# tuffy/libdvd-audio

Measured on AMD Instinct MI355X. Metric: decoded PCM Msamples/s (bit-exact) on 6ch/96k/24b MLP, higher is better.
Workload: dtype int32 (int64 accumulate)

## Files before the change

libdvd-audio_amd/csrc/mlp_hip.hip:

```cpp
#include <hip/hip_runtime.h>
#include <stdint.h>
#include <stdio.h>
#include <stdlib.h>
#include <string.h>
#include <new>
#include <vector>

#include "../../include/dvda_mlp_hip.h"
#include "mlp_step.h"
#include "mlp_decode.h"
#include "mlp_chain.h"
#include "mlp_chain_small.h"
#include "mlp_check.h"
#include "mlp_coop.h"
#include "mlp_index.h"
#include "pcm_unswizzle.h"
#include "wav_pack.h"

using namespace mlp;

#define HIP_TRY(x)                                                                         \
    do {                                                                                   \
        hipError_t e_ = (x);                                                               \
        if (e_ != hipSuccess) {                                                            \
            fprintf(stderr, "dvda_mlp_hip: %s failed: %s (%s:%d)\n", #x, hipGetErrorString(e_), \
                    __FILE__, __LINE__);                                                   \
            return DVDA_HIP_ENODEV;                                                        \
        }                                                                                  \
    } while (0)

constexpr uint32_t EV_RING = 256;
constexpr uint32_t SEQ_ROUND = 1024;

static hipError_t ws_malloc(void **p, size_t bytes)
{
    static const int poison = getenv("DVDA_POISON") ? (int)strtol(getenv("DVDA_POISON"), nullptr, 0) : -1;
    hipError_t e = hipMalloc(p, bytes);
    if (e == hipSuccess && poison >= 0)
        e = hipMemset(*p, poison & 0xFF, bytes);
    return e;
}

struct dvda_mlp_hip_ctx {
    int device;
    uint32_t coop_min_seg;
    uint32_t max_streams, max_segments;
    uint8_t *d_masks;
    uint16_t *d_parts;
    uint64_t masks_cap;
    uint32_t *d_tile_count;
    uint32_t *d_tile_base;
    uint64_t tiles_cap;
    uint64_t *d_cand_off;
    SegRec *d_seg;
    uint32_t *d_seg_frames;
    uint32_t *d_seg_fbase;
    uint32_t *d_seg_status;
    uint32_t *d_seg_rows;
    StreamRec *d_streams;
    uint32_t *d_n_cand;
    uint32_t *d_scan_tmp;
    uint64_t scan_tmp_cap;
    int32_t *d_iir;
    uint32_t *d_mat;
    unsigned long long *d_dbg;
    int32_t *d_fir;
    uint32_t *d_seg_meta;
    uint32_t *d_yield;
    uint32_t *d_seg_check;
    uint32_t *d_cls;
    uint32_t *d_shape_key;
    uint64_t *d_soff, *d_slen;
    uint32_t *d_rank;
    uint32_t *d_sorted_cnt;
    uint32_t *d_sorted_base;
    uint32_t *d_lane_seg;
    DecodeSummary *d_summary;
    DecodeSummary *h_summary;
    hipStream_t st_aux;
    hipEvent_t ev_fork, ev_join;
    uint32_t *d_seq_list;
    uint4 *d_plan;
    uint4 *d_scan4_tmp;
    uint32_t *d_def_list;
    uint32_t *d_head_list;
    uint32_t *d_chain_order;
    uint32_t *d_chain_hist;
    int32_t *d_fb;
    uint32_t fb_slots;
    uint32_t rsv_segs;
    int32_t *d_res;
    uint64_t res_cap;
    uint32_t *d_brec;
    uint64_t brec_cap;
    uint32_t *d_frec;
    uint64_t frec_cap;
    const int32_t *d_init_fir;
    uint32_t iir_lanes;
    const uint8_t *d_bytes;
    uint64_t total_bytes;
    const uint64_t *d_stream_off;
    const uint64_t *d_stream_len;
    uint32_t n_streams;
    uint64_t tiles;
    bool indexed;
    bool small_input;
    bool decoded;
    uint32_t lanes_per_seg;
    uint32_t pcm_layout;
    uint32_t chain_form;
    hipGraphExec_t idx_graph;
    const void *idx_key[4];
    uint64_t idx_key_bytes;
    uint32_t idx_key_streams;
    int idx_graph_state;
    hipEvent_t ev[2 * EV_RING];
    hipEvent_t ev_end[EV_RING];
    uint32_t ev_end_made;
    uint32_t ev_made;
    uint64_t ev_count;
};

static WsCaps ws_caps(const dvda_mlp_hip_ctx *c)
{
    WsCaps w;
    w.res = c->res_cap;
    w.brec = c->brec_cap;
    w.frec = c->frec_cap;
    w.fb = (uint64_t)c->fb_slots * FB_WORDS;
    w.max_seg = c->max_segments;
    w.max_streams = c->max_streams;
    w.lanes = c->iir_lanes;
    w.pad = 0;
    return w;
}

extern "C" int dvda_mlp_hip_bounds_violations(unsigned long long *out4)
{
    if (!out4)
        return DVDA_HIP_EINVAL;
    out4[0] = out4[1] = out4[2] = out4[3] = 0;
#if defined(DVDA_BOUNDS)
    HIP_TRY(hipDeviceSynchronize());
    HIP_TRY(hipMemcpyFromSymbol(out4, HIP_SYMBOL(mlp::g_bounds), 4 * sizeof(unsigned long long)));
    return 1;
#else
    return DVDA_HIP_OK;
#endif
}

static void free_ws(dvda_mlp_hip_ctx *c)
{
    (void)hipFree(c->d_masks);
    (void)hipFree(c->d_parts);
    (void)hipFree(c->d_tile_count);
    (void)hipFree(c->d_tile_base);
    (void)hipFree(c->d_cand_off);
    (void)hipFree(c->d_seg);
    (void)hipFree(c->d_seg_frames);
    (void)hipFree(c->d_seg_fbase);
    (void)hipFree(c->d_seg_status);
    (void)hipFree(c->d_seg_rows);
    (void)hipFree(c->d_streams);
    (void)hipFree(c->d_scan_tmp);
    (void)hipFree(c->d_iir);
    (void)hipFree(c->d_mat);
    (void)hipFree(c->d_dbg);
    (void)hipFree(c->d_fir);
    (void)hipFree(c->d_seg_meta);
    (void)hipFree(c->d_yield);
    (void)hipFree(c->d_seg_check);
    (void)hipFree(c->d_cls);
    (void)hipFree(c->d_shape_key);
    (void)hipFree(c->d_soff);
    (void)hipFree(c->d_slen);
    (void)hipFree(c->d_rank);
    (void)hipFree(c->d_sorted_cnt);
    (void)hipFree(c->d_sorted_base);
    (void)hipFree(c->d_lane_seg);
    (void)hipFree(c->d_summary);
    if (c->h_summary)
        (void)hipHostFree(c->h_summary);
    if (c->st_aux)
        (void)hipStreamDestroy(c->st_aux);
    if (c->ev_fork)
        (void)hipEventDestroy(c->ev_fork);
    if (c->ev_join)
        (void)hipEventDestroy(c->ev_join);
    (void)hipFree(c->d_seq_list);
    (void)hipFree(c->d_plan);
    (void)hipFree(c->d_scan4_tmp);
    (void)hipFree(c->d_def_list);
    (void)hipFree(c->d_head_list);
    (void)hipFree(c->d_chain_order);
    (void)hipFree(c->d_chain_hist);
    (void)hipFree(c->d_fb);
    (void)hipFree(c->d_res);
    (void)hipFree(c->d_brec);
    (void)hipFree(c->d_frec);
    for (uint32_t i = 0; i < c->ev_made; i++)
        (void)hipEventDestroy(c->ev[i]);
    for (uint32_t i = 0; i < c->ev_end_made; i++)
        (void)hipEventDestroy(c->ev_end[i]);
    if (c->idx_graph)
        (void)hipGraphExecDestroy(c->idx_graph);
}

extern "C" const char *dvda_mlp_hip_version(void) { return "dvda-mlp-hip 0.1 (gfx950)"; }

extern "C" int dvda_mlp_hip_create(dvda_mlp_hip_ctx **out, int device, uint32_t max_streams,
                                   uint32_t max_segments)
{
    if (!out || max_streams == 0 || max_segments == 0)
        return DVDA_HIP_EINVAL;
    int ndev = 0;
    if (hipGetDeviceCount(&ndev) != hipSuccess || ndev <= 0 || device < 0 || device >= ndev) {
        fprintf(stderr, "dvda_mlp_hip: no usable HIP device (count=%d, requested=%d)\n", ndev, device);
        return DVDA_HIP_ENODEV;
    }
    HIP_TRY(hipSetDevice(device));
    dvda_mlp_hip_ctx *c = new (std::nothrow) dvda_mlp_hip_ctx();
    if (!c)
        return DVDA_HIP_ENOMEM;
    c->device = device;
    {
        int cus = 0;
        if (hipDeviceGetAttribute(&cus, hipDeviceAttributeMultiprocessorCount, device) != hipSuccess || cus <= 0)
            cus = 256;
        c->coop_min_seg = (uint32_t)cus * 4u * 64u * 7u / 4u;
        if (const char *e = getenv("DVDA_COOP_MIN_SEG"))
            c->coop_min_seg = (uint32_t)strtoul(e, nullptr, 10);
    }
    c->max_streams = max_streams;
    c->max_segments = max_segments;
    c->masks_cap = 0;
    c->tiles_cap = 0;
    c->scan_tmp_cap = 0;
    c->indexed = false;
// ... 20 lines not shown
    alloc((void **)&c->d_seg_status, (ns + 4) * sizeof(uint32_t));
    alloc((void **)&c->d_seg_rows, ns * sizeof(uint32_t));
    alloc((void **)&c->d_streams, (size_t)max_streams * sizeof(StreamRec));
    c->iir_lanes = (uint32_t)(((2 * ns + DEC_THREADS - 1) / DEC_THREADS) * DEC_THREADS);
    alloc((void **)&c->d_iir, (size_t)c->iir_lanes * MAXCH * 16 * sizeof(int32_t));
    alloc((void **)&c->d_mat, (size_t)c->iir_lanes * MAXMAT * 5 * sizeof(uint32_t));
    alloc((void **)&c->d_dbg, 32 * sizeof(unsigned long long));
    alloc((void **)&c->d_fir, (size_t)c->iir_lanes * 6 * 8 * sizeof(int32_t));
    alloc((void **)&c->d_seg_meta, ((size_t)c->iir_lanes + 4) * sizeof(uint32_t));
    alloc((void **)&c->d_yield, ns * sizeof(uint32_t));
    alloc((void **)&c->d_seg_check, 2 * ns * sizeof(uint32_t));
    alloc((void **)&c->d_cls, 4 * sizeof(uint32_t));
    alloc((void **)&c->d_shape_key, (size_t)max_streams * sizeof(uint32_t));
    alloc((void **)&c->d_soff, (size_t)max_streams * sizeof(uint64_t));
    alloc((void **)&c->d_slen, (size_t)max_streams * sizeof(uint64_t));
    alloc((void **)&c->d_rank, (size_t)max_streams * sizeof(uint32_t));
    alloc((void **)&c->d_sorted_cnt, ((size_t)max_streams + 1) * sizeof(uint32_t));
    alloc((void **)&c->d_sorted_base, ((size_t)max_streams + 1) * sizeof(uint32_t));
    alloc((void **)&c->d_lane_seg, ns * sizeof(uint32_t));
    alloc((void **)&c->d_summary, (1 + SUMMARY_PARTS) * sizeof(DecodeSummary));
    alloc((void **)&c->d_seq_list, (size_t)max_streams * sizeof(uint32_t));
    alloc((void **)&c->d_plan, (ns + 5) * sizeof(uint4));
    alloc((void **)&c->d_scan4_tmp, (ns / 1024 + 4) * sizeof(uint4));
    alloc((void **)&c->d_def_list, ns * sizeof(uint32_t));
    alloc((void **)&c->d_head_list, ns * sizeof(uint32_t));
    alloc((void **)&c->d_chain_order, ns * sizeof(uint32_t));
    alloc((void **)&c->d_chain_hist, 2 * CHAIN_BUCKETS * sizeof(uint32_t));
    if (e == hipSuccess)
        e = hipHostMalloc((void **)&c->h_summary, sizeof(DecodeSummary), hipHostMallocDefault);
    if (e == hipSuccess)
        e = hipStreamCreateWithFlags(&c->st_aux, hipStreamNonBlocking);
    if (e == hipSuccess)
        e = hipEventCreateWithFlags(&c->ev_fork, hipEventDisableTiming);
    if (e == hipSuccess)
        e = hipEventCreateWithFlags(&c->ev_join, hipEventDisableTiming);
    if (e == hipSuccess)
        e = hipMemset(c->d_dbg, 0, 32 * sizeof(unsigned long long));
    if (e == hipSuccess)
        e = hipMemset(c->d_seg_meta, 0, (size_t)c->iir_lanes * sizeof(uint32_t));
    for (uint32_t i = 0; e == hipSuccess && i < 2 * EV_RING; i++) {
        e = hipEventCreate(&c->ev[i]);
        if (e == hipSuccess)
            c->ev_made = i + 1;
    }
    for (uint32_t i = 0; e == hipSuccess && i < EV_RING; i++) {
        e = hipEventCreate(&c->ev_end[i]);
        if (e == hipSuccess)
            c->ev_end_made = i + 1;
    }
    if (e != hipSuccess) {
        fprintf(stderr, "dvda_mlp_hip: workspace allocation failed: %s\n", hipGetErrorString(e));
        free_ws(c);
        delete c;
        return DVDA_HIP_ENOMEM;
    }
    *out = c;
    return DVDA_HIP_OK;
}

extern "C" void dvda_mlp_hip_destroy(dvda_mlp_hip_ctx *c)
{
    if (!c)
        return;
    (void)hipSetDevice(c->device);
#if defined(DVDA_BOUNDS)
    if (getenv("DVDA_BOUNDS_REPORT")) {
        unsigned long long v[4] = {0, 0, 0, 0};
        (void)dvda_mlp_hip_bounds_violations(v);
        fprintf(stderr, "dvda_mlp_hip: bounds violations: %llu", v[0]);
        if (v[0])
            fprintf(stderr, " (first: tag %llu index %llu capacity %llu)", v[1], v[2], v[3]);
        fprintf(stderr, "\n");
    }
#endif
    free_ws(c);
    delete c;
}

static int ensure_byte_ws(dvda_mlp_hip_ctx *c, uint64_t total_bytes)
{
    const uint64_t chunks = (total_bytes + 15) / 16 + 4;
    const uint64_t tiles = (chunks + IDX_TILE_CHUNKS - 1) / IDX_TILE_CHUNKS;
    if (chunks > c->masks_cap) {
        (void)hipFree(c->d_masks);
        (void)hipFree(c->d_parts);
        c->d_masks = nullptr;
        c->d_parts = nullptr;
        c->masks_cap = 0;
        if (ws_malloc((void **)&c->d_masks, chunks) != hipSuccess ||
            ws_malloc((void **)&c->d_parts, (chunks + 72) * sizeof(uint16_t)) != hipSuccess)
            return DVDA_HIP_ENOMEM;
        c->masks_cap = chunks;
    }
    {
        uint64_t most = tiles > c->max_segments ? tiles : c->max_segments;
        if (c->max_streams > most)
            most = c->max_streams;
        const uint64_t need = (most + 1023) / 1024 + 2;
        if (need > c->scan_tmp_cap) {
            (void)hipFree(c->d_scan_tmp);
            c->d_scan_tmp = nullptr;
            c->scan_tmp_cap = 0;
            if (ws_malloc((void **)&c->d_scan_tmp, need * sizeof(uint32_t)) != hipSuccess)
                return DVDA_HIP_ENOMEM;
            c->scan_tmp_cap = need;
        }
    }
    if (tiles > c->tiles_cap) {
        (void)hipFree(c->d_tile_count);
        (void)hipFree(c->d_tile_base);
        c->d_tile_count = c->d_tile_base = nullptr;
        c->tiles_cap = 0;
        if (ws_malloc((void **)&c->d_tile_count, (tiles + 1) * sizeof(uint32_t)) != hipSuccess ||
            ws_malloc((void **)&c->d_tile_base, (tiles + 1) * sizeof(uint32_t)) != hipSuccess)
            return DVDA_HIP_ENOMEM;
        c->tiles_cap = tiles;
    }
    return DVDA_HIP_OK;
}

static void exscan(dvda_mlp_hip_ctx *c, hipStream_t st, const uint32_t *in, uint32_t *out, uint32_t n_host,
                   const uint32_t *n_ptr, uint32_t n_cap)
{
    const uint32_t n_max = n_ptr ? n_cap : n_host;
    if (n_max <= 4096) {
        hipLaunchKernelGGL(k_exscan_u32, dim3(1), dim3(1024), 0, st, in, out, n_host, n_ptr, n_cap);
        return;
    }
    const uint32_t blocks = (n_max + 1023) / 1024;
    hipLaunchKernelGGL(k_scan_blocks, dim3(blocks), dim3(1024), 0, st, in, out, c->d_scan_tmp, n_host, n_ptr,
                       n_cap);
    hipLaunchKernelGGL(k_exscan_u32, dim3(1), dim3(1024), 0, st, c->d_scan_tmp, c->d_scan_tmp, blocks,
                       (const uint32_t *)nullptr, blocks);
    hipLaunchKernelGGL(k_scan_add, dim3(blocks), dim3(1024), 0, st, out, c->d_scan_tmp, blocks, n_host, n_ptr,
                       n_cap);
}

__global__ void k_init_streams(StreamRec *s, uint32_t n, uint32_t *seg_status, uint32_t *seg_rows, uint32_t *yield_req,
                               uint32_t *seg_meta, uint32_t n_seg, uint32_t *cls, uint32_t *summary_words)
{
    const uint32_t i = blockIdx.x * blockDim.x + threadIdx.x;
    if (i < 4)
        cls[i] = 0;
    if (i < (1 + SUMMARY_PARTS) * sizeof(DecodeSummary) / sizeof(uint32_t))
        summary_words[i] = 0;
    if (i < n_seg) {
        seg_status[i] = 0;
        seg_rows[i] = 0;
        yield_req[i] = 0;
        seg_meta[2 * (size_t)i] = seg_meta[2 * (size_t)i + 1] = 0;
    }
    if (i < n) {
        StreamRec r;
        r.first_seg = 0xFFFFFFFFu;
        r.n_seg = 0;
        r.sync = 0;
        r.status = 0;
        r.frames = 0;
        r.consumed = 0;
        r.rows = 0;
        s[i] = r;
    }
}

__global__ void k_reset_segments(uint32_t *seg_status, uint32_t *seg_rows, uint32_t *yield_req, uint32_t *seg_meta,
                                 uint32_t n_seg)
{
    const uint32_t i = blockIdx.x * blockDim.x + threadIdx.x;
    if (i < n_seg) {
        seg_status[i] = 0;
        seg_rows[i] = 0;
        yield_req[i] = 0;
        seg_meta[2 * (size_t)i] = seg_meta[2 * (size_t)i + 1] = 0;
    }
}

__device__ __forceinline__ void check_ranges_block(const uint64_t *__restrict__ off, const uint64_t *__restrict__ len,
                                                   uint32_t n, uint64_t total_bytes, uint64_t *__restrict__ soff,
                                                   uint64_t *__restrict__ slen, StreamRec *__restrict__ streams,
                                                   unsigned long long *s_max)
{
    const uint32_t per = (n + 1023u) / 1024u;
    const uint32_t lo = threadIdx.x * per, hi = lo + per < n ? lo + per : n;
    auto end_of = [&](uint32_t i) {
        const uint64_t o = off[i], l = len[i];
        return (o <= total_bytes && l <= total_bytes - o && (o & 15u) == 0) ? o + l : 0;
    };
    unsigned long long m = 0;
    for (uint32_t i = lo; i < hi; i++) {
        const unsigned long long e = end_of(i);
        m = e > m ? e : m;
    }
    s_max[threadIdx.x] = m;
    __syncthreads();
    for (uint32_t d = 1; d < 1024u; d <<= 1) {
        const unsigned long long v = threadIdx.x >= d ? s_max[threadIdx.x - d] : 0ull;
        __syncthreads();
        if (v > s_max[threadIdx.x])
            s_max[threadIdx.x] = v;
        __syncthreads();
    }
    unsigned long long run = threadIdx.x ? s_max[threadIdx.x - 1] : 0ull;
    for (uint32_t i = lo; i < hi; i++) {
        const uint64_t o = off[i], l = len[i];
        const bool ok = (o & 15u) == 0 && o <= total_bytes && l <= total_bytes - o && o >= run;
        const uint64_t so = ok ? o : run;
        soff[i] = so < total_bytes ? so : total_bytes;
        slen[i] = ok ? l : 0;
        if (!ok)
            streams[i].status = ST_ENVELOPE | (1u << 16);
        const unsigned long long e = end_of(i);
        run = e > run ? e : run;
    }
}

__global__ __launch_bounds__(1024) void k_check_ranges(const uint64_t *__restrict__ off, const uint64_t *__restrict__ len,
                                                       uint32_t n, uint64_t total_bytes, uint64_t *__restrict__ soff,
                                                       uint64_t *__restrict__ slen, StreamRec *__restrict__ streams)
{
    __shared__ unsigned long long s_max[1024];
    check_ranges_block(off, len, n, total_bytes, soff, slen, streams, s_max);
}

constexpr uint64_t SMALL_INPUT_BYTES = 4096u * 1024u;

static void enqueue_index(dvda_mlp_hip_ctx *c, hipStream_t st, const uint8_t *d_bytes, uint64_t total_bytes,
                          const uint64_t *d_stream_off, const uint64_t *d_stream_len, uint32_t n_streams)
{
    const uint64_t tiles = c->tiles;
    const uint32_t ms = c->max_segments;
    {
        uint32_t n_init = n_streams > ms ? n_streams : ms;
        if (n_init < 1024)
            n_init = 1024;
        hipLaunchKernelGGL(k_init_streams, dim3((n_init + 255) / 256), dim3(256), 0, st, c->d_streams,
                           n_streams, c->d_seg_status, c->d_seg_rows, c->d_yield, c->d_seg_meta, ms, c->d_cls,
                           reinterpret_cast<uint32_t *>(c->d_summary));
        hipLaunchKernelGGL(k_check_ranges, dim3(1), dim3(1024), 0, st, d_stream_off, d_stream_len, n_streams, total_bytes,
                           c->d_soff, c->d_slen, c->d_streams);
        d_stream_off = c->d_soff;
        d_stream_len = c->d_slen;
    }
    hipLaunchKernelGGL(k_sync_mask, dim3((unsigned)tiles), dim3(IDX_THREADS), 0, st, d_bytes,
                       total_bytes, c->d_masks, c->d_tile_count, c->d_parts);
    exscan(c, st, c->d_tile_count, c->d_tile_base, (uint32_t)tiles, nullptr, (uint32_t)tiles);
    hipLaunchKernelGGL(k_sync_scatter, dim3((unsigned)tiles), dim3(IDX_THREADS), 0, st, c->d_masks,
                       total_bytes, c->d_tile_base, c->d_cand_off, ms);
    hipLaunchKernelGGL(k_chase, dim3((ms + 255) / 256), dim3(256), 0, st, d_bytes, d_stream_off,
                       d_stream_len, n_streams, c->d_cand_off, c->d_n_cand, ms, c->d_seg,
                       c->d_seg_frames, c->d_streams, c->d_cls);
    hipLaunchKernelGGL(k_mark_dead, dim3((ms + 255) / 256), dim3(256), 0, st, d_stream_off, d_stream_len,
                       c->d_n_cand, ms, c->d_seg, c->d_seg_frames, c->d_streams);
    exscan(c, st, c->d_seg_frames, c->d_seg_fbase, 0u, c->d_n_cand, ms);
    const bool pack = !(total_bytes <= SMALL_INPUT_BYTES);
    hipLaunchKernelGGL(k_link, dim3((ms + 255) / 256), dim3(256), 0, st, d_stream_off, d_stream_len,
                       c->d_n_cand, ms, c->d_seg, c->d_seg_fbase, c->d_streams, n_streams, c->d_shape_key,
                       c->d_cls + (pack ? 2 : 3));
    hipStream_t sp = st;
    bool forked = false;
    if (pack && st != nullptr && c->st_aux && hipEventRecord(c->ev_fork, st) == hipSuccess &&
        hipStreamWaitEvent(c->st_aux, c->ev_fork, 0) == hipSuccess) {
        sp = c->st_aux;
        forked = true;
    }
    if (pack) {
    hipLaunchKernelGGL(k_stream_rank, dim3((n_streams + 255) / 256), dim3(256), 0, sp, c->d_shape_key, c->d_streams,
                       n_streams, c->d_rank, c->d_sorted_cnt, c->d_cls + 2);
    exscan(c, sp, c->d_sorted_cnt, c->d_sorted_base, n_streams, nullptr, n_streams);
    (void)hipMemsetAsync(c->d_lane_seg, 0xFF, (size_t)ms * sizeof(uint32_t), sp);
    hipLaunchKernelGGL(k_lane_perm, dim3((ms + 255) / 256), dim3(256), 0, sp, c->d_seg, c->d_streams, c->d_n_cand, ms,
                       c->d_rank, c->d_sorted_base, c->d_cls + 2, c->d_lane_seg);
    }
    hipLaunchKernelGGL(k_au_check, dim3((unsigned)(((uint64_t)ms * CHK_GROUP + CHK_THREADS - 1) / CHK_THREADS)),
                       dim3(CHK_THREADS), 0, st, d_bytes, c->d_parts, c->d_seg, c->d_n_cand, ms, c->d_streams, c->d_seg_check);
    if (forked) {
        (void)hipEventRecord(c->ev_join, sp);
        (void)hipStreamWaitEvent(st, c->ev_join, 0);
    }
}

extern "C" int dvda_mlp_hip_index(dvda_mlp_hip_ctx *c, const uint8_t *d_bytes, uint64_t total_bytes,
                                  const uint64_t *d_stream_off, const uint64_t *d_stream_len,
                                  uint32_t n_streams, void *stream_)
{
    if (!c || !d_bytes || !d_stream_off || !d_stream_len || n_streams == 0 || total_bytes == 0)
        return DVDA_HIP_EINVAL;
    if (n_streams > c->max_streams)
        return DVDA_HIP_ECAPACITY;
    if (((uintptr_t)d_bytes & 15) != 0)
        return DVDA_HIP_EINVAL;
    hipStream_t st = (hipStream_t)stream_;
    HIP_TRY(hipSetDevice(c->device));
    int rc = ensure_byte_ws(c, total_bytes);
    if (rc)
        return rc;
    c->d_bytes = d_bytes;
    c->total_bytes = total_bytes;
    c->d_stream_off = d_stream_off;
    c->d_stream_len = d_stream_len;
    c->n_streams = n_streams;
    const uint64_t chunks = (total_bytes + 15) / 16;
    const uint64_t tiles = (chunks + IDX_TILE_CHUNKS - 1) / IDX_TILE_CHUNKS;
    c->tiles = tiles;
    c->d_n_cand = c->d_tile_base + tiles;

    c->small_input = total_bytes <= SMALL_INPUT_BYTES;
    const bool same = c->idx_graph_state > 0 && c->idx_key[0] == d_bytes && c->idx_key[1] == d_stream_off &&
                      c->idx_key[2] == d_stream_len && c->idx_key[3] == (const void *)st &&
                      c->idx_key_bytes == total_bytes && c->idx_key_streams == n_streams;
    if (c->idx_graph_state == 2 && same) {
        if (hipGraphLaunch(c->idx_graph, st) == hipSuccess) {
            c->indexed = true;
            c->decoded = false;
            return DVDA_HIP_OK;
        }
        (void)hipGetLastError();
        c->idx_graph_state = -1;
    } else if (c->idx_graph_state == 1 && same && st != nullptr) {
        hipGraph_t g = nullptr;
        bool ok = hipStreamBeginCapture(st, hipStreamCaptureModeThreadLocal) == hipSuccess;
        if (ok) {
            enqueue_index(c, st, d_bytes, total_bytes, d_stream_off, d_stream_len, n_streams);
            ok = hipStreamEndCapture(st, &g) == hipSuccess && g != nullptr;
        }
        if (ok) {
            if (c->idx_graph) {
                (void)hipGraphExecDestroy(c->idx_graph);
                c->idx_graph = nullptr;
            }
            ok = hipGraphInstantiate(&c->idx_graph, g, nullptr, nullptr, 0) == hipSuccess;
// ... 492 lines not shown
    if (e == hipSuccess)
        e = hipMemcpy(d_w, host_widths, n * sizeof(int32_t), hipMemcpyHostToDevice);
    if (e == hipSuccess) {
        hipLaunchKernelGGL(k_selftest_bits, dim3(1), dim3(64), 0, 0, d_b, n_bytes, d_w, n, d_o, resident);
        e = hipMemcpy(host_out, d_o, n * sizeof(int64_t), hipMemcpyDeviceToHost);
    }
    (void)hipFree(d_b);
    (void)hipFree(d_w);
    (void)hipFree(d_o);
    return e == hipSuccess ? DVDA_HIP_OK : DVDA_HIP_ENODEV;
}

extern "C" int dvda_mlp_hip_set_initial_fir(dvda_mlp_hip_ctx *c, const int32_t *d_init_fir)
{
    if (!c)
        return DVDA_HIP_EINVAL;
    c->d_init_fir = d_init_fir;
    return DVDA_HIP_OK;
}

extern "C" int dvda_mlp_hip_segment_info(dvda_mlp_hip_ctx *c, uint32_t segment, dvda_mlp_segment_info *info,
                                         void *stream_)
{
    if (!c || !info)
        return DVDA_HIP_EINVAL;
    if (!c->indexed)
        return DVDA_HIP_ESTATE;
    if (segment >= c->max_segments)
        return DVDA_HIP_EINVAL;
    HIP_TRY(hipSetDevice(c->device));
    HIP_TRY(hipStreamSynchronize((hipStream_t)stream_));
    SegRec r;
    uint32_t rows = 0, st = 0;
    HIP_TRY(hipMemcpy(&r, c->d_seg + segment, sizeof(r), hipMemcpyDeviceToHost));
    HIP_TRY(hipMemcpy(&rows, c->d_seg_rows + segment, sizeof(rows), hipMemcpyDeviceToHost));
    HIP_TRY(hipMemcpy(&st, c->d_seg_status + segment, sizeof(st), hipMemcpyDeviceToHost));
    info->offset = r.off;
    info->end = r.end;
    info->stream = r.stream;
    info->mlp_frames = r.nframes;
    info->pcm_frames = rows;
    info->status = st | r.flags;
    return DVDA_HIP_OK;
}

extern "C" int dvda_mlp_hip_segment_fir(dvda_mlp_hip_ctx *c, uint32_t segment, int32_t *host_fir, void *stream_)
{
    if (!c || !host_fir)
        return DVDA_HIP_EINVAL;
    if (!c->indexed)
        return DVDA_HIP_ESTATE;
    const uint32_t L = 2;
    if ((uint64_t)segment * L + L > c->iir_lanes)
        return DVDA_HIP_EINVAL;
    HIP_TRY(hipSetDevice(c->device));
    HIP_TRY(hipStreamSynchronize((hipStream_t)stream_));
    memset(host_fir, 0, 2 * 48 * sizeof(int32_t));
    for (uint32_t s = 0; s < L; s++) {
        HIP_TRY(hipMemcpy2D(host_fir + s * 48, sizeof(int32_t), c->d_fir + (size_t)segment * L + s,
                            (size_t)c->iir_lanes * sizeof(int32_t), sizeof(int32_t), 48,
                            hipMemcpyDeviceToHost));
    }
    return DVDA_HIP_OK;
}

struct StepDesc {
    SegRec seg;
    StreamRec streams;
    uint32_t seg_fbase[2];
    uint32_t n_seg;
    uint32_t state_valid;
    uint64_t out_off, out_stride;
    uint32_t cls[4];
};
constexpr size_t STEP_DESC_BYTES = 256;
static_assert(sizeof(StepDesc) <= STEP_DESC_BYTES, "the descriptor fits its place");
static_assert(sizeof(dvda_mlp_step_result) == sizeof(CoopResult), "the result record is the kernel's");
constexpr size_t STEP_PCM_BYTES = (size_t)DVDA_STEP_MAX_UNITS * 160u * 6u * 4u;

struct dvda_mlp_hip_stepper {
    int device;
    hipStream_t st;
    uint8_t *d_in;
    uint8_t *d_masks;
    uint16_t *d_parts;
    uint32_t *d_tile_count;
    uint32_t *d_small;
    DecodeSummary *d_summary;
    CoopState *d_state;
    uint8_t *d_out;
    uint8_t *h_in, *h_out;
};

__global__ __launch_bounds__(IDX_THREADS) void k_step_check(const uint8_t *__restrict__ bytes, uint32_t total_bytes,
                                                            uint16_t *__restrict__ parts, const StepDesc *__restrict__ d,
                                                            uint32_t *__restrict__ seg_check)
{
    __shared__ __attribute__((aligned(16))) uint8_t s_slice[16 * 256];
    __shared__ __attribute__((aligned(16))) uint8_t s_log[256];
    __shared__ __attribute__((aligned(16))) uint8_t s_exp[512];
    for (int i = threadIdx.x; i < 16 * 256 / 16; i += IDX_THREADS)
        reinterpret_cast<uint4 *>(s_slice)[i] = reinterpret_cast<const uint4 *>(d_chk.slice)[i];
    for (int i = threadIdx.x; i < 256 / 16; i += IDX_THREADS)
        reinterpret_cast<uint4 *>(s_log)[i] = reinterpret_cast<const uint4 *>(d_chk.log)[i];
    for (int i = threadIdx.x; i < 512 / 16; i += IDX_THREADS)
        reinterpret_cast<uint4 *>(s_exp)[i] = reinterpret_cast<const uint4 *>(d_chk.exp)[i];
    __syncthreads();
    const uint32_t n_chunks = (total_bytes + 15u) >> 4;
    for (uint32_t chunk = threadIdx.x; chunk < n_chunks; chunk += IDX_THREADS) {
        uint32_t part;
        (void)mask_chunk(bytes, total_bytes, chunk, s_slice, part);
        parts[chunk] = (uint16_t)part;
    }
    __threadfence_block();
    __syncthreads();
    if (threadIdx.x < (uint32_t)CHK_GROUP)
        au_check_group(0, threadIdx.x, bytes, parts, &d->seg, &d->streams, seg_check, s_slice, s_log, s_exp);
}

extern "C" void dvda_mlp_hip_stepper_destroy(dvda_mlp_hip_stepper *s)
{
    if (!s)
        return;
    (void)hipSetDevice(s->device);
    if (s->st)
        (void)hipStreamSynchronize(s->st);
    (void)hipFree(s->d_masks);
    (void)hipFree(s->d_parts);
    (void)hipFree(s->d_tile_count);
    (void)hipFree(s->d_small);
    (void)hipFree(s->d_summary);
    (void)hipFree(s->d_state);
    (void)hipHostFree(s->h_in);
    (void)hipHostFree(s->h_out);
    if (s->st)
        (void)hipStreamDestroy(s->st);
    free(s);
}

extern "C" int dvda_mlp_hip_stepper_create(dvda_mlp_hip_stepper **out, int device)
{
    if (!out)
        return DVDA_HIP_EINVAL;
    *out = nullptr;
    int n_dev = 0;
    if (hipGetDeviceCount(&n_dev) != hipSuccess || device < 0 || device >= n_dev)
        return DVDA_HIP_ENODEV;
    dvda_mlp_hip_stepper *s = (dvda_mlp_hip_stepper *)calloc(1, sizeof(*s));
    if (!s)
        return DVDA_HIP_ENOMEM;
    s->device = device;
    const size_t in_bytes = STEP_DESC_BYTES + DVDA_STEP_MAX_BYTES + 128;
    const size_t chunks = (DVDA_STEP_MAX_BYTES + 128) / 16 + 8;
    const size_t out_bytes = sizeof(CoopResult) + STEP_PCM_BYTES;
    bool ok = hipSetDevice(device) == hipSuccess && hipStreamCreateWithFlags(&s->st, hipStreamNonBlocking) == hipSuccess &&
              hipMalloc((void **)&s->d_masks, chunks) == hipSuccess &&
              hipMalloc((void **)&s->d_parts, chunks * 2) == hipSuccess &&
              hipMalloc((void **)&s->d_tile_count, 4 * sizeof(uint32_t)) == hipSuccess &&
              hipMalloc((void **)&s->d_small, 16 * sizeof(uint32_t)) == hipSuccess &&
              hipMalloc((void **)&s->d_summary, (1 + SUMMARY_PARTS) * sizeof(DecodeSummary)) == hipSuccess &&
              hipMalloc((void **)&s->d_state, 2 * sizeof(CoopState)) == hipSuccess &&
              hipHostMalloc((void **)&s->h_in, in_bytes, hipHostMallocMapped | hipHostMallocCoherent) == hipSuccess &&
              hipHostMalloc((void **)&s->h_out, out_bytes, hipHostMallocMapped | hipHostMallocCoherent) == hipSuccess &&
              hipHostGetDevicePointer((void **)&s->d_in, s->h_in, 0) == hipSuccess &&
              hipHostGetDevicePointer((void **)&s->d_out, s->h_out, 0) == hipSuccess;
    ok = ok && hipMemset(s->d_state, 0, 2 * sizeof(CoopState)) == hipSuccess &&
         hipMemset(s->d_summary, 0, (1 + SUMMARY_PARTS) * sizeof(DecodeSummary)) == hipSuccess &&
         hipMemset(s->d_small, 0, 16 * sizeof(uint32_t)) == hipSuccess;
    if (!ok) {
        dvda_mlp_hip_stepper_destroy(s);
        return DVDA_HIP_ENODEV;
    }
    memset(s->h_in, 0, in_bytes);
    memset(s->h_out, 0, out_bytes);
    *out = s;
    return DVDA_HIP_OK;
}

extern "C" int dvda_mlp_hip_stepper_step(dvda_mlp_hip_stepper *s, const uint8_t *bytes, size_t len, uint32_t n_units,
                                         uint32_t packed_sync, int fresh, const dvda_mlp_step_result **res,
                                         const int32_t **pcm, uint64_t *stride, unsigned *channels)
{
    if (!s || !bytes || !res || !pcm || !stride || len == 0 || n_units == 0)
        return DVDA_HIP_EINVAL;
    if (len > DVDA_STEP_MAX_BYTES || n_units > DVDA_STEP_MAX_UNITS)
        return DVDA_HIP_ECAPACITY;
    const uint32_t rpa = rows_per_au((packed_sync >> 8) & 0xFu);
    const uint32_t nch = channel_count((packed_sync >> 16) & 0x1Fu);
    if (rpa == 0 || nch == 0)
        return DVDA_HIP_EINVAL;
    HIP_TRY(hipSetDevice(s->device));
    const uint64_t rows_cap = (uint64_t)n_units * rpa;
    StepDesc *d = reinterpret_cast<StepDesc *>(s->h_in);
    memset(d, 0, sizeof(*d));
    d->seg.off = 0;
    d->seg.end = len;
    d->seg.stream = 0;
    d->seg.nframes = n_units;
    d->seg.flags = SEG_STREAMING;
    d->seg.sync = packed_sync;
    d->seg.ndrop = 0;
    d->seg.prev = 0xFFFFFFFFu;
    d->streams.first_seg = 0;
    d->streams.n_seg = 1;
    d->streams.sync = packed_sync;
    d->seg_fbase[0] = 0;
    d->seg_fbase[1] = n_units;
    d->n_seg = 1;
    d->state_valid = fresh ? 0u : 1u;
    d->out_off = 0;
    d->out_stride = rows_cap;
    d->cls[0] = d->cls[1] = 1;
    uint8_t *hb = s->h_in + STEP_DESC_BYTES;
    memcpy(hb, bytes, len);
    memset(hb + len, 0, 128);
    const StepDesc *dd = reinterpret_cast<const StepDesc *>(s->d_in);
    const uint8_t *d_bytes = s->d_in + STEP_DESC_BYTES;
    hipLaunchKernelGGL(k_step_check, dim3(1), dim3(IDX_THREADS), 0, s->st, d_bytes, (uint32_t)len, s->d_parts, dd, s->d_small);
    DecodeArgs a;
    memset(&a, 0, sizeof(a));
    a.bytes = d_bytes;
    a.total_bytes = len;
    a.seg = &dd->seg;
    a.seg_fbase = dd->seg_fbase;
    a.n_seg_ptr = &dd->n_seg;
    a.max_seg = 1;
    a.streams = const_cast<StreamRec *>(&dd->streams);
    a.pcm = reinterpret_cast<int32_t *>(s->d_out + sizeof(CoopResult));
    a.out_off = &dd->out_off;
    a.out_stride = &dd->out_stride;
    a.seg_status = s->d_small + 2;
    a.seg_rows = s->d_small + 3;
    a.yield_req = s->d_small + 4;
    a.seg_meta = s->d_small + 5;
    a.seg_check = s->d_small;
    a.total_lanes = 2;
    a.summary = s->d_summary;
    a.cls = dd->cls;
    a.coop = 64;
// ... 149 lines not shown
```

libdvd-audio_amd/csrc/mlp_index.h:

```cpp
#pragma once
#include <hip/hip_runtime.h>
#include <stdint.h>
#include "mlp_tables.h"

namespace mlp {

struct SegRec {
    uint64_t off;
    uint64_t end;
    uint32_t stream;
    uint32_t nframes;
    uint32_t flags;
    uint32_t sync;
    uint32_t ndrop;
    uint32_t prev;
};
constexpr uint32_t SYNC_PARAMS = 0x00FFFFFFu;
constexpr uint32_t MAX_DROP = 64;

struct StreamRec {
    uint32_t first_seg;
    uint32_t n_seg;
    uint32_t sync;
    uint32_t status;
    uint64_t frames;
    uint64_t consumed;
    uint64_t rows;
};

constexpr int IDX_THREADS = 256;
constexpr int IDX_CHUNKS_PER_THREAD = 16;
constexpr int IDX_TILE_CHUNKS = IDX_THREADS * IDX_CHUNKS_PER_THREAD;

__device__ __forceinline__ uint32_t ld_u8(const uint8_t *p, uint64_t i) { return p[i]; }

__device__ __forceinline__ bool sync_frame_at(const uint8_t *b, uint64_t p, uint64_t limit)
{
    if (p + 32 > limit)
        return false;
    const uint32_t size = 2u * (((ld_u8(b, p) & 0x0Fu) << 8) | ld_u8(b, p + 1));
    if (size < 32)
        return false;
    if (ld_u8(b, p + 4) != 0xF8 || ld_u8(b, p + 5) != 0x72 || ld_u8(b, p + 6) != 0x6F ||
        ld_u8(b, p + 7) != 0xBB)
        return false;
    const uint32_t count = ld_u8(b, p + 20) >> 4;
    return count == 1 || count == 2;
}

__device__ __forceinline__ uint64_t ld_hdr8(const uint8_t *b, uint64_t p)
{
    const uint16_t *h = reinterpret_cast<const uint16_t *>(b + p);
    return (uint64_t)h[0] | ((uint64_t)h[1] << 16) | ((uint64_t)h[2] << 32) | ((uint64_t)h[3] << 48);
}

__device__ __forceinline__ bool sync_frame_hdr(const uint8_t *b, uint64_t p, uint64_t limit, uint64_t hdr)
{
    if (p + 32 > limit)
        return false;
    const uint32_t size = 2u * ((((uint32_t)hdr & 0x0Fu) << 8) | (((uint32_t)hdr >> 8) & 0xFFu));
    if (size < 32 || (uint32_t)(hdr >> 32) != 0xBB6F72F8u)
        return false;
    const uint32_t count = ld_u8(b, p + 20) >> 4;
    return count == 1 || count == 2;
}

__device__ __forceinline__ uint32_t packed_sync_at(const uint8_t *b, uint64_t p)
{
    return (ld_u8(b, p + 8) >> 4) | ((ld_u8(b, p + 8) & 0xFu) << 4) | ((ld_u8(b, p + 9) >> 4) << 8) |
           ((ld_u8(b, p + 9) & 0xFu) << 12) | ((ld_u8(b, p + 11) & 0x1Fu) << 16) | ((ld_u8(b, p + 20) >> 4) << 24);
}

__device__ const CheckTables d_chk = make_check();

__device__ __forceinline__ uint32_t mask_chunk(const uint8_t *__restrict__ bytes, uint64_t total_bytes, uint64_t chunk,
                                               const uint8_t *s_slice, uint32_t &part)
{
    const uint4 *q = reinterpret_cast<const uint4 *>(bytes) + chunk;
    const uint4 a = q[0], c = q[1];
    uint32_t w[8] = {a.x, a.y, a.z, a.w, c.x, c.y, c.z, c.w};
    uint32_t m = 0;
    uint32_t any = 0;
#pragma unroll
    for (int k = 1; k <= 4; k++) {
        const uint32_t y = w[k] ^ 0x72F872F8u;
        any |= (y - 0x00010001u) & ~y & 0x80008000u;
    }
    if (__builtin_expect(any != 0, 0)) {
#pragma unroll
        for (int j = 0; j < 8; j++) {
            const int h = j + 2;
            const uint32_t lo = (h & 1) ? (w[h >> 1] >> 16) : (w[h >> 1] & 0xFFFFu);
            const uint32_t hi = ((h + 1) & 1) ? (w[(h + 1) >> 1] >> 16) : (w[(h + 1) >> 1] & 0xFFFFu);
            if (lo == 0x72F8u && hi == 0xBB6Fu) {
                if (sync_frame_at(bytes, chunk * 16 + 2 * j, total_bytes))
                    m |= 1u << j;
            }
        }
    }
    uint32_t c0 = 0;
#pragma unroll
    for (int k = 0; k < 4; k++)
        c0 ^= s_slice[(15 - 4 * k) * 256 + (w[k] & 0xFFu)] ^ s_slice[(14 - 4 * k) * 256 + ((w[k] >> 8) & 0xFFu)] ^
              s_slice[(13 - 4 * k) * 256 + ((w[k] >> 16) & 0xFFu)] ^ s_slice[(12 - 4 * k) * 256 + (w[k] >> 24)];
    uint32_t px = w[0] ^ w[1] ^ w[2] ^ w[3];
    px ^= px >> 16;
    px = (px ^ (px >> 8)) & 0xFFu;
    part = c0 | (px << 8);
    return m;
}

__global__ __launch_bounds__(IDX_THREADS) void k_sync_mask(const uint8_t *__restrict__ bytes,
                                                           uint64_t total_bytes,
                                                           uint8_t *__restrict__ masks,
                                                           uint32_t *__restrict__ tile_count,
                                                           uint16_t *__restrict__ parts)
{
    __shared__ uint32_t s_cnt[IDX_THREADS / 64];
    __shared__ uint8_t s_slice[16 * 256];
    for (int i = threadIdx.x; i < 16 * 256 / 16; i += IDX_THREADS)
        reinterpret_cast<uint4 *>(s_slice)[i] = reinterpret_cast<const uint4 *>(d_chk.slice)[i];
    __syncthreads();
    const uint64_t n_chunks = (total_bytes + 15) >> 4;
    const uint64_t tile0 = (uint64_t)blockIdx.x * IDX_TILE_CHUNKS;
    uint32_t cnt = 0;
    for (int k = 0; k < IDX_CHUNKS_PER_THREAD; k++) {
        const uint64_t chunk = tile0 + (uint64_t)k * IDX_THREADS + threadIdx.x;
        if (chunk >= n_chunks)
            break;
        uint32_t part;
        const uint32_t m = mask_chunk(bytes, total_bytes, chunk, s_slice, part);
        masks[chunk] = (uint8_t)m;
        cnt += __popc(m);
        parts[chunk] = (uint16_t)part;
    }
    for (int o = 32; o > 0; o >>= 1)
        cnt += __shfl_down(cnt, o, 64);
    if ((threadIdx.x & 63) == 0)
        s_cnt[threadIdx.x >> 6] = cnt;
    __syncthreads();
    if (threadIdx.x == 0) {
        uint32_t t = 0;
        for (int i = 0; i < IDX_THREADS / 64; i++)
            t += s_cnt[i];
        tile_count[blockIdx.x] = t;
    }
}

__global__ __launch_bounds__(1024) void k_exscan_u32(const uint32_t *__restrict__ in,
                                                     uint32_t *__restrict__ out, uint32_t n_host,
                                                     const uint32_t *__restrict__ n_ptr,
                                                     uint32_t n_cap)
{
    __shared__ uint32_t s_part[1024];
    uint32_t n = n_ptr ? *n_ptr : n_host;
    if (n > n_cap)
        n = n_cap;
    const uint32_t per = (n + 1023) / 1024;
    const uint32_t lo = threadIdx.x * per;
    const uint32_t hi = lo + per < n ? lo + per : n;
    uint32_t sum = 0;
    for (uint32_t i = lo; i < hi; i++)
        sum += in[i];
    s_part[threadIdx.x] = sum;
    __syncthreads();
    for (int o = 1; o < 1024; o <<= 1) {
        uint32_t v = threadIdx.x >= (uint32_t)o ? s_part[threadIdx.x - o] : 0;
        __syncthreads();
        s_part[threadIdx.x] += v;
        __syncthreads();
    }
    uint32_t run = threadIdx.x ? s_part[threadIdx.x - 1] : 0;
    for (uint32_t i = lo; i < hi; i++) {
        const uint32_t v = in[i];
        out[i] = run;
        run += v;
    }
    if (threadIdx.x == 1023)
        out[n] = s_part[1023];
}

__global__ __launch_bounds__(1024) void k_scan_blocks(const uint32_t *__restrict__ in,
                                                      uint32_t *__restrict__ out,
                                                      uint32_t *__restrict__ block_sum, uint32_t n_host,
                                                      const uint32_t *__restrict__ n_ptr, uint32_t n_cap)
{
    __shared__ uint32_t s_v[1024];
    uint32_t n = n_ptr ? *n_ptr : n_host;
    if (n > n_cap)
        n = n_cap;
    const uint32_t i = blockIdx.x * 1024 + threadIdx.x;
    const uint32_t v = i < n ? in[i] : 0;
    s_v[threadIdx.x] = v;
    __syncthreads();
    for (int o = 1; o < 1024; o <<= 1) {
        const uint32_t t = threadIdx.x >= (uint32_t)o ? s_v[threadIdx.x - o] : 0;
        __syncthreads();
        s_v[threadIdx.x] += t;
        __syncthreads();
    }
    if (i < n)
        out[i] = s_v[threadIdx.x] - v;
    if (threadIdx.x == 1023)
        block_sum[blockIdx.x] = s_v[1023];
}

__global__ __launch_bounds__(1024) void k_scan_add(uint32_t *__restrict__ out,
                                                   const uint32_t *__restrict__ block_base,
                                                   uint32_t n_blocks, uint32_t n_host,
                                                   const uint32_t *__restrict__ n_ptr, uint32_t n_cap)
{
    uint32_t n = n_ptr ? *n_ptr : n_host;
    if (n > n_cap)
        n = n_cap;
    const uint32_t i = blockIdx.x * 1024 + threadIdx.x;
    if (i < n)
        out[i] += block_base[blockIdx.x];
    if (i == 0)
        out[n] = block_base[n_blocks];
}

__global__ __launch_bounds__(IDX_THREADS) void k_sync_scatter(const uint8_t *__restrict__ masks,
                                                              uint64_t total_bytes,
                                                              const uint32_t *__restrict__ tile_base,
                                                              uint64_t *__restrict__ cand_off,
                                                              uint32_t max_cand)
{
    __shared__ uint32_t s_wave[IDX_THREADS / 64];
    const uint64_t n_chunks = (total_bytes + 15) >> 4;
    const uint64_t first = (uint64_t)blockIdx.x * IDX_TILE_CHUNKS +
                           (uint64_t)threadIdx.x * IDX_CHUNKS_PER_THREAD;
    static_assert(IDX_CHUNKS_PER_THREAD == 16, "one 16-byte load of mask bytes per thread");
    uint8_t m[IDX_CHUNKS_PER_THREAD];
    uint32_t cnt = 0;
    if (first + IDX_CHUNKS_PER_THREAD <= n_chunks) {
        const uint4 q = *reinterpret_cast<const uint4 *>(masks + first);
        const uint32_t w[4] = {q.x, q.y, q.z, q.w};
#pragma unroll
        for (int k = 0; k < IDX_CHUNKS_PER_THREAD; k++)
            m[k] = (uint8_t)(w[k >> 2] >> (8 * (k & 3)));
        cnt = __popc(q.x) + __popc(q.y) + __popc(q.z) + __popc(q.w);
    } else {
#pragma unroll
        for (int k = 0; k < IDX_CHUNKS_PER_THREAD; k++) {
            m[k] = (first + k < n_chunks) ? masks[first + k] : 0;
            cnt += __popc((uint32_t)m[k]);
        }
    }
    uint32_t inc = cnt;
#pragma unroll
    for (int o = 1; o < 64; o <<= 1) {
        const uint32_t v = __shfl_up(inc, o, 64);
        if ((int)(threadIdx.x & 63) >= o)
            inc += v;
    }
    if ((threadIdx.x & 63) == 63)
        s_wave[threadIdx.x >> 6] = inc;
    __syncthreads();
    uint32_t before = 0;
    for (uint32_t w = 0; w < (threadIdx.x >> 6); w++)
        before += s_wave[w];
    uint32_t at = tile_base[blockIdx.x] + before + inc - cnt;
    if (cnt == 0)
        return;
#pragma unroll
    for (int k = 0; k < IDX_CHUNKS_PER_THREAD; k++) {
        uint32_t mk = m[k];
        while (mk) {
            const int j = __ffs(mk) - 1;
            mk &= mk - 1;
            if (at < max_cand)
                cand_off[at] = (first + k) * 16 + 2 * j;
            at++;
        }
    }
}

__device__ __forceinline__ uint32_t find_stream(const uint64_t *__restrict__ stream_off,
                                                uint32_t n_streams, uint64_t p)
{
    uint32_t lo = 0, hi = n_streams;
    while (hi - lo > 1) {
        const uint32_t mid = (lo + hi) >> 1;
        if (stream_off[mid] <= p)
            lo = mid;
        else
            hi = mid;
    }
    return lo;
}

constexpr uint32_t SEG_DEAD = 1u << 24;

__device__ __forceinline__ void chase_one(uint32_t i, const uint8_t *__restrict__ bytes,
                                          const uint64_t *__restrict__ stream_off,
                                          const uint64_t *__restrict__ stream_len, uint32_t n_streams,
                                          const uint64_t *__restrict__ cand_off, SegRec *__restrict__ seg,
                                          uint32_t *__restrict__ seg_frames, StreamRec *__restrict__ streams,
                                          uint32_t *__restrict__ cls)
{
    const uint64_t off = cand_off[i];
    const uint32_t s = find_stream(stream_off, n_streams, off);
    const uint64_t s_begin = stream_off[s];
    const uint64_t s_end = s_begin + stream_len[s];
    SegRec r;
    r.off = off;
    r.stream = s;
    r.flags = 0;
    r.nframes = 0;
    r.sync = 0;
    r.ndrop = 0;
    r.prev = 0xFFFFFFFFu;
    uint64_t p = off;
    const bool outside = off >= s_end;
    if (outside) {
        r.flags = SEG_DEAD;
        r.end = off;
    } else if ((off - s_begin) & 1) {
        r.flags = 1u << 16;
        r.end = off;
    } else if (!sync_frame_at(bytes, off, s_end)) {
        r.flags = SEG_DEAD;
        r.end = off;
    } else {
        r.sync = packed_sync_at(bytes, off);
        const bool own = sync_frame_at(bytes, s_begin, s_end) &&
                         ((packed_sync_at(bytes, s_begin) ^ r.sync) & SYNC_PARAMS) == 0;
        uint32_t n = 0;
        uint64_t hdr = ld_hdr8(bytes, p);
        for (;;) {
// ... 287 lines not shown
```

Baseline: 238,700.

## Drop global sync-mask buffer; stash per-tile candidate slots, recompute on overflow

The sync-mask kernel no longer writes a per-chunk mask byte array to global memory. It builds the masks in LDS, computes per-tile prefix offsets, and writes up to 64 candidate offsets per tile into a compact slot buffer. The scatter kernel copies those slots directly when a tile has few candidates and only recomputes candidates from the raw bytes for dense tiles. This removes the mask write/read traffic, but it adds an extra block-level scan and an LDS buffer in the mask kernel, plus a costly recompute path for dense tiles.

```diff
diff --git a/libdvd-audio_amd/csrc/mlp_hip.hip b/libdvd-audio_amd/csrc/mlp_hip.hip
--- a/libdvd-audio_amd/csrc/mlp_hip.hip
+++ b/libdvd-audio_amd/csrc/mlp_hip.hip
@@ -45,10 +45,10 @@
     int device;
     uint32_t coop_min_seg;
     uint32_t max_streams, max_segments;
-    uint8_t *d_masks;
     uint16_t *d_parts;
     uint64_t masks_cap;
     uint32_t *d_tile_count;
+    uint32_t *d_slots;
     uint32_t *d_tile_base;
     uint64_t tiles_cap;
     uint64_t *d_cand_off;
@@ -151,9 +151,9 @@
 
 static void free_ws(dvda_mlp_hip_ctx *c)
 {
-    (void)hipFree(c->d_masks);
     (void)hipFree(c->d_parts);
     (void)hipFree(c->d_tile_count);
+    (void)hipFree(c->d_slots);
     (void)hipFree(c->d_tile_base);
     (void)hipFree(c->d_cand_off);
     (void)hipFree(c->d_seg);
@@ -340,13 +340,10 @@
     const uint64_t chunks = (total_bytes + 15) / 16 + 4;
     const uint64_t tiles = (chunks + IDX_TILE_CHUNKS - 1) / IDX_TILE_CHUNKS;
     if (chunks > c->masks_cap) {
-        (void)hipFree(c->d_masks);
         (void)hipFree(c->d_parts);
-        c->d_masks = nullptr;
         c->d_parts = nullptr;
         c->masks_cap = 0;
-        if (ws_malloc((void **)&c->d_masks, chunks) != hipSuccess ||
-            ws_malloc((void **)&c->d_parts, (chunks + 72) * sizeof(uint16_t)) != hipSuccess)
+        if (ws_malloc((void **)&c->d_parts, (chunks + 72) * sizeof(uint16_t)) != hipSuccess)
             return DVDA_HIP_ENOMEM;
         c->masks_cap = chunks;
     }
@@ -367,10 +364,12 @@
     if (tiles > c->tiles_cap) {
         (void)hipFree(c->d_tile_count);
         (void)hipFree(c->d_tile_base);
-        c->d_tile_count = c->d_tile_base = nullptr;
+        (void)hipFree(c->d_slots);
+        c->d_tile_count = c->d_tile_base = c->d_slots = nullptr;
         c->tiles_cap = 0;
         if (ws_malloc((void **)&c->d_tile_count, (tiles + 1) * sizeof(uint32_t)) != hipSuccess ||
-            ws_malloc((void **)&c->d_tile_base, (tiles + 1) * sizeof(uint32_t)) != hipSuccess)
+            ws_malloc((void **)&c->d_tile_base, (tiles + 1) * sizeof(uint32_t)) != hipSuccess ||
+            ws_malloc((void **)&c->d_slots, tiles * CAND_SLOT * sizeof(uint32_t)) != hipSuccess)
             return DVDA_HIP_ENOMEM;
         c->tiles_cap = tiles;
     }
@@ -500,10 +499,10 @@
         d_stream_len = c->d_slen;
     }
     hipLaunchKernelGGL(k_sync_mask, dim3((unsigned)tiles), dim3(IDX_THREADS), 0, st, d_bytes,
-                       total_bytes, c->d_masks, c->d_tile_count, c->d_parts);
+                       total_bytes, c->d_slots, c->d_tile_count, c->d_parts);
     exscan(c, st, c->d_tile_count, c->d_tile_base, (uint32_t)tiles, nullptr, (uint32_t)tiles);
-    hipLaunchKernelGGL(k_sync_scatter, dim3((unsigned)tiles), dim3(IDX_THREADS), 0, st, c->d_masks,
-                       total_bytes, c->d_tile_base, c->d_cand_off, ms);
+    hipLaunchKernelGGL(k_sync_scatter, dim3((unsigned)tiles), dim3(IDX_THREADS), 0, st, d_bytes,
+                       total_bytes, c->d_tile_count, c->d_slots, c->d_tile_base, c->d_cand_off, ms);
     hipLaunchKernelGGL(k_chase, dim3((ms + 255) / 256), dim3(256), 0, st, d_bytes, d_stream_off,
                        d_stream_len, n_streams, c->d_cand_off, c->d_n_cand, ms, c->d_seg,
                        c->d_seg_frames, c->d_streams, c->d_cls);
@@ -1162,7 +1161,6 @@
     int device;
     hipStream_t st;
     uint8_t *d_in;
-    uint8_t *d_masks;
     uint16_t *d_parts;
     uint32_t *d_tile_count;
     uint32_t *d_small;
@@ -1205,7 +1203,6 @@
     (void)hipSetDevice(s->device);
     if (s->st)
         (void)hipStreamSynchronize(s->st);
-    (void)hipFree(s->d_masks);
     (void)hipFree(s->d_parts);
     (void)hipFree(s->d_tile_count);
     (void)hipFree(s->d_small);
@@ -1234,7 +1231,6 @@
     const size_t chunks = (DVDA_STEP_MAX_BYTES + 128) / 16 + 8;
     const size_t out_bytes = sizeof(CoopResult) + STEP_PCM_BYTES;
     bool ok = hipSetDevice(device) == hipSuccess && hipStreamCreateWithFlags(&s->st, hipStreamNonBlocking) == hipSuccess &&
-              hipMalloc((void **)&s->d_masks, chunks) == hipSuccess &&
               hipMalloc((void **)&s->d_parts, chunks * 2) == hipSuccess &&
               hipMalloc((void **)&s->d_tile_count, 4 * sizeof(uint32_t)) == hipSuccess &&
               hipMalloc((void **)&s->d_small, 16 * sizeof(uint32_t)) == hipSuccess &&
diff --git a/libdvd-audio_amd/csrc/mlp_index.h b/libdvd-audio_amd/csrc/mlp_index.h
--- a/libdvd-audio_amd/csrc/mlp_index.h
+++ b/libdvd-audio_amd/csrc/mlp_index.h
@@ -32,6 +32,8 @@
 constexpr int IDX_CHUNKS_PER_THREAD = 16;
 constexpr int IDX_TILE_CHUNKS = IDX_THREADS * IDX_CHUNKS_PER_THREAD;
 
+constexpr uint32_t CAND_SLOT = 64;
+
 __device__ __forceinline__ uint32_t ld_u8(const uint8_t *p, uint64_t i) { return p[i]; }
 
 __device__ __forceinline__ bool sync_frame_at(const uint8_t *b, uint64_t p, uint64_t limit)
@@ -73,12 +75,9 @@
 
 __device__ const CheckTables d_chk = make_check();
 
-__device__ __forceinline__ uint32_t mask_chunk(const uint8_t *__restrict__ bytes, uint64_t total_bytes, uint64_t chunk,
-                                               const uint8_t *s_slice, uint32_t &part)
-{
-    const uint4 *q = reinterpret_cast<const uint4 *>(bytes) + chunk;
-    const uint4 a = q[0], c = q[1];
-    uint32_t w[8] = {a.x, a.y, a.z, a.w, c.x, c.y, c.z, c.w};
+__device__ __forceinline__ uint32_t chunk_candidates(const uint8_t *__restrict__ bytes, uint64_t total_bytes, uint64_t chunk,
+                                                     const uint32_t (&w)[8])
+{
     uint32_t m = 0;
     uint32_t any = 0;
 #pragma unroll
@@ -98,6 +97,16 @@
             }
         }
     }
+    return m;
+}
+
+__device__ __forceinline__ uint32_t mask_chunk(const uint8_t *__restrict__ bytes, uint64_t total_bytes, uint64_t chunk,
+                                               const uint8_t *s_slice, uint32_t &part)
+{
+    const uint4 *q = reinterpret_cast<const uint4 *>(bytes) + chunk;
+    const uint4 a = q[0], c = q[1];
+    const uint32_t w[8] = {a.x, a.y, a.z, a.w, c.x, c.y, c.z, c.w};
+    const uint32_t m = chunk_candidates(bytes, total_bytes, chunk, w);
     uint32_t c0 = 0;
 #pragma unroll
     for (int k = 0; k < 4; k++)
@@ -112,38 +121,57 @@
 
 __global__ __launch_bounds__(IDX_THREADS) void k_sync_mask(const uint8_t *__restrict__ bytes,
                                                            uint64_t total_bytes,
-                                                           uint8_t *__restrict__ masks,
+                                                           uint32_t *__restrict__ slots,
                                                            uint32_t *__restrict__ tile_count,
                                                            uint16_t *__restrict__ parts)
 {
-    __shared__ uint32_t s_cnt[IDX_THREADS / 64];
+    __shared__ uint32_t s_wave[IDX_THREADS / 64];
     __shared__ uint8_t s_slice[16 * 256];
+    __shared__ __attribute__((aligned(16))) uint8_t s_m[IDX_TILE_CHUNKS];
     for (int i = threadIdx.x; i < 16 * 256 / 16; i += IDX_THREADS)
         reinterpret_cast<uint4 *>(s_slice)[i] = reinterpret_cast<const uint4 *>(d_chk.slice)[i];
+    static_assert(IDX_CHUNKS_PER_THREAD == 16, "one 16-byte LDS access of mask bytes per thread");
+    reinterpret_cast<uint4 *>(s_m)[threadIdx.x] = make_uint4(0, 0, 0, 0);
     __syncthreads();
     const uint64_t n_chunks = (total_bytes + 15) >> 4;
     const uint64_t tile0 = (uint64_t)blockIdx.x * IDX_TILE_CHUNKS;
-    uint32_t cnt = 0;
     for (int k = 0; k < IDX_CHUNKS_PER_THREAD; k++) {
         const uint64_t chunk = tile0 + (uint64_t)k * IDX_THREADS + threadIdx.x;
         if (chunk >= n_chunks)
             break;
         uint32_t part;
         const uint32_t m = mask_chunk(bytes, total_bytes, chunk, s_slice, part);
-        masks[chunk] = (uint8_t)m;
-        cnt += __popc(m);
+        s_m[k * IDX_THREADS + threadIdx.x] = (uint8_t)m;
         parts[chunk] = (uint16_t)part;
     }
-    for (int o = 32; o > 0; o >>= 1)
-        cnt += __shfl_down(cnt, o, 64);
-    if ((threadIdx.x & 63) == 0)
-        s_cnt[threadIdx.x >> 6] = cnt;
     __syncthreads();
-    if (threadIdx.x == 0) {
-        uint32_t t = 0;
-        for (int i = 0; i < IDX_THREADS / 64; i++)
-            t += s_cnt[i];
-        tile_count[blockIdx.x] = t;
+    const uint4 q = reinterpret_cast<const uint4 *>(s_m)[threadIdx.x];
+    const uint32_t cnt = __popc(q.x) + __popc(q.y) + __popc(q.z) + __popc(q.w);
+    uint32_t inc = cnt;
+#pragma unroll
+    for (int o = 1; o < 64; o <<= 1) {
+        const uint32_t v = __shfl_up(inc, o, 64);
+        if ((int)(threadIdx.x & 63) >= o)
+            inc += v;
+    }
+    if ((threadIdx.x & 63) == 63)
+        s_wave[threadIdx.x >> 6] = inc;
+    __syncthreads();
+    uint32_t at = inc - cnt, total = 0;
+    for (uint32_t w = 0; w < IDX_THREADS / 64; w++) {
+        at += w < (threadIdx.x >> 6) ? s_wave[w] : 0u;
+        total += s_wave[w];
+    }
+    if (threadIdx.x == 0)
+        tile_count[blockIdx.x] = total;
+    if (cnt == 0 || at >= CAND_SLOT)
+        return;
+    const uint32_t w4[4] = {q.x, q.y, q.z, q.w};
+#pragma unroll
+    for (int k = 0; k < IDX_CHUNKS_PER_THREAD; k++) {
+        for (uint32_t mk = (w4[k >> 2] >> (8 * (k & 3))) & 0xFFu; mk && at < CAND_SLOT; mk &= mk - 1, at++)
+            slots[(uint64_t)blockIdx.x * CAND_SLOT + at] =
+                (threadIdx.x * IDX_CHUNKS_PER_THREAD + (uint32_t)k) * 16u + 2u * (uint32_t)(__ffs(mk) - 1);
     }
 }
 
@@ -220,32 +248,39 @@
         out[n] = block_base[n_blocks];
 }
 
-__global__ __launch_bounds__(IDX_THREADS) void k_sync_scatter(const uint8_t *__restrict__ masks,
+__global__ __launch_bounds__(IDX_THREADS) void k_sync_scatter(const uint8_t *__restrict__ bytes,
                                                               uint64_t total_bytes,
+                                                              const uint32_t *__restrict__ tile_count,
+                                                              const uint32_t *__restrict__ slots,
                                                               const uint32_t *__restrict__ tile_base,
                                                               uint64_t *__restrict__ cand_off,
                                                               uint32_t max_cand)
 {
     __shared__ uint32_t s_wave[IDX_THREADS / 64];
+    const uint32_t n = tile_count[blockIdx.x];
+    if (n == 0)
+        return;
+    if (n <= CAND_SLOT) {
+        const uint32_t at = tile_base[blockIdx.x] + threadIdx.x;
+        if (threadIdx.x < n && at < max_cand)
+            cand_off[at] = (uint64_t)blockIdx.x * IDX_TILE_CHUNKS * 16u + slots[(uint64_t)blockIdx.x * CAND_SLOT + threadIdx.x];
+        return;
+    }
     const uint64_t n_chunks = (total_bytes + 15) >> 4;
     const uint64_t first = (uint64_t)blockIdx.x * IDX_TILE_CHUNKS +
                            (uint64_t)threadIdx.x * IDX_CHUNKS_PER_THREAD;
-    static_assert(IDX_CHUNKS_PER_THREAD == 16, "one 16-byte load of mask bytes per thread");
     uint8_t m[IDX_CHUNKS_PER_THREAD];
     uint32_t cnt = 0;
-    if (first + IDX_CHUNKS_PER_THREAD <= n_chunks) {
-        const uint4 q = *reinterpret_cast<const uint4 *>(masks + first);
-        const uint32_t w[4] = {q.x, q.y, q.z, q.w};
-#pragma unroll
-        for (int k = 0; k < IDX_CHUNKS_PER_THREAD; k++)
-            m[k] = (uint8_t)(w[k >> 2] >> (8 * (k & 3)));
-        cnt = __popc(q.x) + __popc(q.y) + __popc(q.z) + __popc(q.w);
-    } else {
-#pragma unroll
-        for (int k = 0; k < IDX_CHUNKS_PER_THREAD; k++) {
-            m[k] = (first + k < n_chunks) ? masks[first + k] : 0;
-            cnt += __popc((uint32_t)m[k]);
-        }
+#pragma unroll
+    for (int k = 0; k < IDX_CHUNKS_PER_THREAD; k++) {
+        m[k] = 0;
+        if (first + k < n_chunks) {
+            const uint4 *q = reinterpret_cast<const uint4 *>(bytes) + first + k;
+            const uint4 a = q[0], c = q[1];
+            const uint32_t w[8] = {a.x, a.y, a.z, a.w, c.x, c.y, c.z, c.w};
+            m[k] = (uint8_t)chunk_candidates(bytes, total_bytes, first + k, w);
+        }
+        cnt += __popc((uint32_t)m[k]);
     }
     uint32_t inc = cnt;
 #pragma unroll
```

Result: no change. 240,800 (median of 6 runs) (+0.9%).
